# andrekuros/Multi-UAV-TA-gym-env

Hardware: AMD Instinct MI355X
Metric: env-steps/sec at N parallel envs, WPS_hard 16x32; 1/2/4/8 GPU (higher is better)
Workload: dtype f64

## Files before the change

### multi-uav-ta-gym-env_amd/csrc/muavta_state.h

```cpp
#pragma once
#include <stdint.h>

#include "../../include/muavta.h"


enum {
  MUAVTA_ERR_NONE = 0,
  MUAVTA_ERR_TASK_SLOTS = 1,
  MUAVTA_ERR_QUEUE = 2,
  MUAVTA_ERR_EVENTS = 3,
  MUAVTA_ERR_PENDING = 4,
  MUAVTA_ERR_POSITION = 5,
  MUAVTA_ERR_ESCORTS = 6,
  MUAVTA_ERR_LSAP = 7,
};

enum { TF_ESCORT = 1, TF_COUNTED = 2, TF_REACHED = 4, TF_ELIGIBLE = 8, TF_DEADLINE = 16,
       TF_KNOWN_ALL = 32  };

struct DevParams {
  int32_t n_agents, n_tasks , max_tasks , n_threats;
  int32_t n_agent_groups, agent_type[MUAVTA_MAX_GROUPS], agent_count[MUAVTA_MAX_GROUPS];
  int32_t n_task_groups, task_type[MUAVTA_MAX_GROUPS], task_count[MUAVTA_MAX_GROUPS];
  int32_t n_threat_groups, threat_type[MUAVTA_MAX_GROUPS], threat_count[MUAVTA_MAX_GROUPS];
  int32_t max_time_steps, multiple_tasks_per_agent, early_terminate, capability_mask, saturate_mask,
      include_time_windows, threat_delay, hard_windows, window_length, burst_mode, burst_size,
      dual_region_bursts, share_knowledge, escort_enabled, num_obstacles, random_init_pos,
      escort_required_agents , commit_horizon;
  uint32_t escort_mask;
  double speed[7];
  double threat_prob;
  double reward_norm_factor;
  double sense_sq_bound;
  double fail_rate, arrival_rate, dynamic_idle_penalty, sense_radius, miss_penalty, on_time_bonus,
      reassign_penalty, escort_radius, escort_requirement, escort_intercept_radius, mutual_support_radius;
  double rw[8];
  double escort_sq_bound;
  double inv_mts, inv_max_tasks;
  int32_t slot_cap;
  int32_t rw_plain;
};

template <int A_, int T_, int H_, int R_, int E_, int Q_, bool REGC_ = false, bool OTFC_ = false, bool SLIM_ = false, bool TIMES_LDS_ = false>
struct Tile {
  static constexpr bool TIMES_LDS = TIMES_LDS_;
  static constexpr bool SLIM = SLIM_;
  static constexpr bool REGC = REGC_;
  static constexpr bool OTFC = OTFC_;
  static constexpr bool NO_COST_TILE = REGC_ || OTFC_;
  static constexpr int A = A_;
  static constexpr int T = T_;
  static constexpr int H = H_;
  static constexpr int R = R_;
  static constexpr int E = E_;
  static constexpr int Q = Q_;
  static constexpr int KW = (T_ + 31) / 32;
  static constexpr int MIN_WAVES = A_ > 32 ? 2 : 4;
  static_assert(A_ <= 64 && T_ <= 128 && H_ <= 64, "ids of agents / slots / threats are stored in int8");
};

template <int A> struct KnowMask { typedef uint64_t type; };
template <> struct KnowMask<16> { typedef uint16_t type; };
template <> struct KnowMask<24> { typedef uint32_t type; };
template <int A> struct BucketMask { typedef unsigned long long type; };
template <> struct BucketMask<16> { typedef uint32_t type; };
template <> struct BucketMask<24> { typedef uint32_t type; };

typedef int8_t i8;
typedef int16_t i16;
typedef uint8_t u8;

template <int A, int T, bool HERE> struct QueueSide {
  double a_nfx[A], a_nfy[A], a_nft[A];
  double t_org[T], t_done[T];
  double area[3][3];
};
template <int A, int T> struct QueueSide<A, T, false> {};

template <int T, bool HERE> struct TaskTimes {
  double t_init[T], t_dtime[T];
};
template <int T> struct TaskTimes<T, false> {};

template <int T> struct TaskReqs {
  double t_cur[6][T], t_alloc[6][T];
};
template <class TL>
struct alignas(16) EnvCold : QueueSide<TL::A, TL::T, TL::SLIM>, TaskReqs<TL::T>, TaskTimes<TL::T, !TL::TIMES_LDS> {
  enum { A = TL::A, T = TL::T, Q = TL::Q };
  double a_qtime[A][Q];
  double obst[8][3];
};

template <class TL>
struct alignas(16) EnvState : QueueSide<TL::A, TL::T, !TL::SLIM>, TaskTimes<TL::T, TL::TIMES_LDS> {
  enum { A = TL::A, T = TL::T, H = TL::H, R = TL::R, E = TL::E, Q = TL::Q, KW = TL::KW };
  double a_px[A], a_py[A];
  double a_dist[A];
  double a_caps[6][A];
  double t_px[T], t_py[T];
  double h_px[H], h_py[H];
  typename BucketMask<A>::type t_bucket[T];
  uint32_t known[A][KW];
  uint32_t free_slots[KW];
  i16 act_index[A];
  i16 a_qid[A][Q];
  i16 a_task_start[A], a_fail[A], a_last_id[A], a_commit[A];
  i16 a_gone[A];
  i16 t_id[T];
  i16 t_created[T], t_deadline[T], t_prot_id[T];
  i16 h_task_id[H], h_tdeadline[H];
  i16 ev_arg[E], dev_arg[E];
  i16 pend_time[R], pend_id[R];
  i16 esc_id[A], esc_pid[A];
  typename KnowMask<A>::type pend_know[R];
  i8 a_qslot[A][Q];
  i8 a_qlen[A];
  i8 a_state[A], a_acap[A], a_type[A], a_name[A], a_reeval[A], a_last_slot[A];
  i8 t_status[T], t_type[T], t_required[T];
  u8 t_flags[T], t_elig[T];
  i8 t_threat[T];
  i8 t_prot_agent[T], t_prot_slot[T];
  i8 t_ndet[T];
  u8 t_order[T];
  u8 open_slot[T];
  u8 t_row[T];
  i8 h_status[H];
  i8 h_target[H], h_mission[H], h_intercept[H];
  i8 h_task_slot[H], h_det_slot[H], h_acap[H], h_type[H], h_group[H];
  u8 h_tflags[H];
  u8 h_order[H];
  i8 g_next[MUAVTA_MAX_GROUPS], g_end[MUAVTA_MAX_GROUPS];
  u8 ev_tag[E];
  u8 dev_tag[E];
  u8 pend_slot[R];
  i8 esc_agent[A], esc_slot[A], esc_pslot[A];
  i8 act_agent[A], act_slot[A];
  unsigned long long esc_mask;
  double F_Reward, total_distance, last_reward, step_reward;
  double r_time_penalty, r_alloc;
  int32_t time_steps, conclusion_time, n_order, n_open, n_active_threats, n_events, n_dev, n_pending, n_escorts, n_act;
  int32_t next_task_id, n_reached, n_retired_empty_buckets;
  int32_t n_reallocations, n_task_switches, n_arrivals, n_missed_windows, n_on_time, n_windowed_tasks,
      idle_reserve_steps, burst_region_toggle, escort_requests, escort_completed, escort_failed,
      escort_required_steps, escort_covered_steps, protection_breaches, threats_intercepted, recon_losses,
      escort_losses, mutual_support_engagements, protected_rec_completed;
  int32_t pending_reset, terminated, truncated, error, did_reset;
  int32_t last_plan_step, n_replans, n_calls;
  int32_t gate_step;
  uint32_t rng_idx[4];
  uint32_t rng_win[4][8];
  uint32_t rng_win_at[4];
  int32_t times_dirty;
  int32_t obs_rows;
  int32_t list_stale;
};

#ifndef MUAVTA_TIMES_LDS
#define MUAVTA_TIMES_LDS 1
#endif
typedef Tile<16, 40, 16, 48, 40, 10, true, false, false, MUAVTA_TIMES_LDS != 0> Tile16;
#ifndef MUAVTA_TILE24_SLIM
#define MUAVTA_TILE24_SLIM 1
#endif
typedef Tile<24, 48, 24, 88, 32, 12, true, false, MUAVTA_TILE24_SLIM != 0> Tile24;
typedef Tile<64, 128, 48, 128, 96, 12, true, true> Tile64;

#define MUAVTA_REL_ROW 29
#define MUAVTA_RNG_STREAMS 4
#define MUAVTA_RNG_WORDS 1248
```

### multi-uav-ta-gym-env_amd/csrc/sim/step.inc

```
  DEV double np_sum_wave(const double* d, int n) {
    double res;
    if (n < 8) {
      res = 0.;
      for (int i = 0; i < n; i++) res += d[i];
      return res;
    }
    const int body = n - (n % 8);
    double r = 0.;
    if (lane < 8) {
      r = d[lane];
      for (int i = 8 + lane; i < body; i += 8) r += d[i];
    }
    r = r + dpp_xchg(r, 0);
    r = r + dpp_xchg(r, 1);
    r = r + dpp_xchg(r, 2);
    res = readlane_f64(r, 0);
    for (int i = body; i < n; i++) res += d[i];
    return res;
  }

  DEV double np_sum_lanes16(double d, int n_) {
    const int n = __builtin_amdgcn_readfirstlane(n_);
    double res;
    if (n < 8) {
      res = 0.;
      for (int i = 0; i < n; i++) res += readlane_f64(d, i);
      return res;
    }
    const int body = n - (n % 8);
    double r = d;
    if (body == 16) {
      const int lo = __builtin_amdgcn_update_dpp(0, __double2loint(d), 0x108, 0xf, 0xf, true);
      const int hi = __builtin_amdgcn_update_dpp(0, __double2hiint(d), 0x108, 0xf, 0xf, true);
      r = d + __hiloint2double(hi, lo);
    }
    r = r + dpp_xchg(r, 0);
    r = r + dpp_xchg(r, 1);
    r = r + dpp_xchg(r, 2);
    res = readlane_f64(r, 0);
    for (int i = body; i < n; i++) res += readlane_f64(d, i);
    return res;
  }

  DEV void step(bool write_obs_flag) {
    PROF(0);
    in_step = true;
    uint32_t rng_words = 0;
    if (!ABL(0)) { rng_refill(); rng_words = rng_prefetch_issue(); }
    PROF(1);
    double prev_x = 0, prev_y = 0;
    if (lane < P.n_agents) { prev_x = S.a_px[lane]; prev_y = S.a_py[lane]; }
    lds_sync();
    double r_action = 0, r_distance = 0, r_quality = 0, r_squality = 0;
    {
      const int nev = S.n_events;
      for (int k = lane; k < nev; k += WG) { S.dev_tag[k] = S.ev_tag[k]; S.dev_arg[k] = S.ev_arg[k]; }
      tnow += 1;
      if (lane == 0) { S.step_reward = 0; S.time_steps = tnow; S.n_dev = nev; S.n_events = 0; }
      lds_sync();
      int last_arg = -1000;
      bool last_changed = true;
      if (!ABL(1))
      for (int k = 0; k < nev; k++)
        if (S.dev_tag[k] == MUAVTA_EV_RESET_ALLOCATION) {
          const int arg = S.dev_arg[k];
          if (arg == last_arg && !last_changed) continue;
          last_changed = release_all_tasks_coop(arg);
          last_arg = arg;
        }
    }
    PROF(2);
    if (!ABL(2))
    for (;;) {
      if (S.n_act > 0 && !apply_actions_parallel(r_action, r_distance, r_squality)) {
        precompute_actions();
        lds_sync();
        PROF(33);
        if (lane == 0) step_serial_a(r_action, r_distance, r_quality, r_squality);
        cold_sync();
      }
      if (!more_agent || stage_more() == 0) break;
    }
    PROF(3);
    for (int start = ABL(3) ? P.n_agents : 0; start < P.n_agents;) {
      bool popped = false;
      const int first = move_parallel(start, popped);
      if (popped) cold_sync(); else lds_sync();
      PROF(26);
#ifdef MUAVTA_PROF
      PROF_COUNT(40, 1000); if (first < P.n_agents) PROF_COUNT(41, 1000);
#endif
      if (first >= P.n_agents) break;
      if (lane == 0) step_serial_move(first, first + 1, r_quality);
      cold_sync();
      PROF(4);
      start = first + 1;
    }
    double dist_sum = 0.0;
    if (!ABL(4)) {
      double d = 0.0;
      if (lane < P.n_agents) {
        double dx = S.a_px[lane] - prev_x, dy = S.a_py[lane] - prev_y;
        d = fsqrt(dx * dx + dy * dy);
        S.a_dist[lane] += d;
        if constexpr (A > 16) X.u[lane] = d;
      }
      if constexpr (A <= 16) dist_sum = np_sum_lanes16(d, P.n_agents);
      else { lds_sync(); dist_sum = np_sum_wave(X.u, P.n_agents); }
    }
    if (!ABL(0)) rng_prefetch_commit(rng_words);
    PROF(5);
    if (!ABL(5)) {
    precompute_threat_targets();
    if (lane == 0) step_serial_b(dist_sum);
    lds_sync();
    }
    if (!ABL(5))
    {
      unsigned long long livemask = 0ull;
      if (lane == 0) X.retarget_h = -1;
      if (!P.escort_enabled) {
        const unsigned long long em = update_threats_parallel(0, livemask, true);
        lds_sync();
        PROF(23);
        PROF_COUNT(54, 1000);
        if (em) {
          PROF_COUNT(55, 1000 * __popcll(em));
          for (unsigned long long m = em; m; m &= m - 1ull) {
            if (lane == 0) update_threats_serial(__ffsll((long long)m) - 1, livemask);
            lds_sync();
            resolve_retarget();
          }
        }
      } else
      for (int start = 0;;) {
        const int first = (int)update_threats_parallel(start, livemask, false);
        lds_sync();
        PROF(23);
        PROF_COUNT(54, 1000);
        if (first >= S.n_active_threats) break;
        PROF_COUNT(55, 1000);
        if (lane == 0) update_threats_serial(first, livemask);
        lds_sync();
        resolve_retarget();
        start = first + 1;
      }
      if (lane == 0) step_serial_b2();
    }
    lds_sync();
    if (!ABL(6)) {
    if (P.escort_enabled) sync_escorts_coop();
    PROF(6);
    sense_parallel();
    lds_sync();
    }
    PROF(7);
    if (!ABL(7))
    {
      bool due = false, expiring = false, idle = false, resp = false, blocking = false;
      if (!ABL(12)) for (int k = lane; k < S.n_pending; k += WG) due |= tnow >= S.pend_time[k];
      auto scan_slots = [&]() {
        expiring = false; blocking = false;
        for (int k = lane; k < S.n_order; k += WG) {
          const int s = S.t_order[k];
          const int fl = S.t_flags[s], st = S.t_status[s], dl = S.t_deadline[s], ty = S.t_type[s];
          expiring |= (fl & TF_DEADLINE) && st != 2 && tnow > dl;
          blocking |= !((fl & TF_ESCORT) || ty == MUAVTA_DET || ty == MUAVTA_HOLD || st == 2);
        }
        idle = false; resp = false;
        if (lane < P.n_agents && S.a_state[lane] != -1) { idle = S.a_qlen[lane] == 0; resp = !idle; }
      };
      if (!ABL(12)) scan_slots();
      const bool any_due = __ballot(due) != 0ull;
      const bool any_exp = P.hard_windows && __ballot(expiring) != 0ull;
      PROF(28);
      if (any_due || any_exp) process_lists_coop(any_due, any_exp);
      lds_sync();
      PROF(29);
      if (any_exp) scan_slots();
      const int n_idle = __popcll(__ballot(idle));
      const bool responding = __ballot(resp) != 0ull;
      const bool all_done_tasks = __ballot(blocking) == 0ull;
      PROF(32);
      if (!ABL(11) && lane == 0) step_serial_c(r_action, r_distance, r_quality, r_squality, n_idle, responding, all_done_tasks);
    }
    lds_sync();
    PROF(8);
    if (!ABL(8)) finish_step_parallel(true);
    PROF(9);
  }

  DEV void displacement(double px, double py, double ux, double uy, double speed, double& ddx, double& ddy) {
    double avx, avy;
    avoid_obstacles(px, py, ux, uy, avx, avy);
    double mx = ux + avx, my = uy + avy;
    norm_vector(mx, my);
    ddx = mx * speed; ddy = my * speed;
  }
  DEV int move_parallel(int start, bool& popped) {
    const int a = lane;
    const bool in_fleet = a >= start && a < P.n_agents;
    const int ai = in_fleet ? a : 0;
    const int st0 = S.a_state[ai], fail_at = S.a_fail[ai], ts0 = S.a_task_start[ai], qlen = S.a_qlen[ai], reeval = S.a_reeval[ai];
    const int atype = S.a_type[ai];
    const int last_id = S.a_last_id[ai], last_slot = S.a_last_slot[ai], head_id_ = S.a_qid[ai][0], head_slot = S.a_qslot[ai][0];
    double px = S.a_px[ai], py = S.a_py[ai];
    const bool live = in_fleet && st0 != -1;
    int cid = 0, cs = -1;
    if (reeval) { cid = last_id; cs = last_slot; }
    else if (qlen > 0) { cid = head_id_; cs = head_slot; }
    const int csi = cs >= 0 ? cs : 0;
    const int tid_at = S.t_id[csi], tstat = S.t_status[csi], ty = S.t_type[csi];
    const double tpx = S.t_px[csi], tpy = S.t_py[csi];
    bool evt = false, pop_head = false;
    int new_st = 0, new_ts = 0;
    double ddx = 0.0, ddy = 0.0;
    if (live) {
      if (fail_at == tnow) {
        evt = true;
      } else {
        const double speed = speed_of(atype);
        new_st = st0; new_ts = ts0;
        const bool retired = cid != 0 && (!(cs >= 0 && tid_at == cid) || tstat == 2);
        const bool to_task = cid != 0 && !retired;
        const bool idle_check = new_st == 0 && !reeval && qlen == 0;
        const bool to_base = !to_task && (idle_check || new_st == 3);
        if (retired) pop_head = true;
        if (to_task || to_base) {
          const double tx = to_task ? tpx : BASE_X, ty_ = to_task ? tpy : BASE_Y;
          const double dx = tx - px, dy = ty_ - py;
          const double dist = norm2(dx, dy);
          double ux = 0, uy = 0;
          const bool zero = to_task ? (fabs(dist) < 1e-12) : (dist == 0);
          if (!zero) { const double r = frcp_nr(dist); ux = fdiv_r(dx, dist, r); uy = fdiv_r(dy, dist, r); }
          double ndx, ndy;
          displacement(px, py, ux, uy, speed, ndx, ndy);
          if (to_task) {
            const double engage = engage_range(atype);
            if (new_st == 1) {
              if (ty == MUAVTA_INT) {
                if (dist < engage) evt = true;
                else { ddx = ndx; ddy = ndy; }
              } else if (dist < speed) {
                new_st = 2; new_ts = tnow;
                px = tpx; py = tpy;
              } else { ddx = ndx; ddy = ndy; }
            } else if (new_st == 2) {
              if (ty == MUAVTA_INT && dist >= engage) new_st = 1;
              if (new_ts == -1) {
                new_ts = tnow;
                px = tpx; py = tpy;
              } else if ((tnow - new_ts) >= task_duration(ty) && ty != MUAVTA_HOLD && ty != MUAVTA_DEF &&
                         ty != MUAVTA_INT && ty != MUAVTA_DET) {
                evt = true;
              }
            }
          } else {
            if (idle_check && dist > speed + 5) new_st = 3;
            if (new_st == 3) {
              if (dist < speed + 5) new_st = 0;
              else { ddx = ndx; ddy = ndy; }
            }
          }
        }
      }
    }
    const unsigned long long em = __ballot(evt);
    const int first = em ? __ffsll((long long)em) - 1 : P.n_agents;
    PROF(34);
    popped = __ballot(live && a < first && pop_head) != 0ull;
    if (live && a < first) {
      if (pop_head) {
        des_allocate(a, cid);
        S.a_reeval[a] = 0;
        S.a_last_id[a] = -1; S.a_last_slot[a] = -1;
      }
      S.a_state[a] = new_st;
      S.a_task_start[a] = new_ts;
      px = px + ddx; py = py + ddy;
      S.a_px[a] = fmin(fmax(px, 0.0), AREA_W);
      S.a_py[a] = fmin(fmax(py, 0.0), AREA_H);
    }
    return first;
  }

  DEV double* act_f(int k) { return X.cost + k * A; }
  DEV void precompute_actions() {
    cold_sync();
    const int k = lane;
    if (k >= S.n_act) return;
    const int a = S.act_agent[k], s = S.act_slot[k];
    X.remaining[k] = -1;
    if (a < 0 || s < 0 || S.a_state[a] == -1) return;
    const double px = S.a_px[a], py = S.a_py[a], tx = S.t_px[s], ty = S.t_py[s];
    double d_old = 0;
    if (S.a_qlen[a] > 0) { const int hs = S.a_qslot[a][0]; d_old = norm2(px - S.t_px[hs], py - S.t_py[hs]); }
    act_f(0)[k] = d_old;
    act_f(1)[k] = norm2(px - tx, py - ty);
    act_f(2)[k] = fdiv(norm2(qs().a_nfx[a] - tx, qs().a_nfy[a] - ty), speed_of(S.a_type[a]));
    const int n = S.a_qlen[a];
    double total;
    if (n >= 1) { const int ps = S.a_qslot[a][n - 1]; total = norm2(tx - S.t_px[ps], ty - S.t_py[ps]); }
    else total = norm2(tx - px, ty - py);
    act_f(3)[k] = -div_coord(total);
    bool dup = false;
#pragma clang loop unroll(disable) vectorize(disable)
    for (int q = 0; q < k; q++) dup |= S.act_agent[q] == a;
    if (!dup) X.remaining[k] = a;
  }
```

### multi-uav-ta-gym-env_amd/csrc/sim/world.inc

```
  DEV bool threat_spawn_step() const { return tnow > 40 && tnow % 10 == 0; }
  DEV void precompute_threat_targets() {
    if (!threat_spawn_step() || P.dual_region_bursts) return;
    const int nA = P.n_agents;
    for (int g = 0; g < P.n_threat_groups; g++) {
      const int start = S.g_next[g], left = S.g_end[g] - start;
      int cnt = P.burst_mode ? (P.burst_size < left ? P.burst_size : left) : (left > 0 ? 1 : 0);
      if (cnt <= 0) continue;
      const int chunk = Scratch<TL>::COSTN / nA;
      for (int c0 = 0; c0 < cnt; c0 += chunk) {
        const int cn = cnt - c0 < chunk ? cnt - c0 : chunk;
        for (int p = lane; p < cn * nA; p += WG) {
          const int c = p / nA, a = p - c * nA, h = start + c0 + c;
          const int st = S.a_state[a];
          X.cost[p] = (h < H && st != -1 && st != 4) ? norm2(S.a_px[a] - S.h_px[h], S.a_py[a] - S.h_py[h]) : __builtin_huge_val();
        }
        lds_sync();
        for (int c = lane; c < cn; c += WG) {
          double minF = __builtin_huge_val(), minW = __builtin_huge_val();
          int cF = -1, cW = -1;
          for (int a = 0; a < nA; a++) {
            const double d = X.cost[c * nA + a];
            const int st = S.a_state[a];
            if (st != -1 && st != 4) {
              if (is_fighter(S.a_type[a])) { if (d < minF) { minF = d; cF = a; } }
              else { if (d < minW) { minW = d; cW = a; } }
            }
          }
          if (start + c0 + c < H) X.roundT[start + c0 + c] = cW >= 0 ? cW : cF;
        }
        lds_sync();
      }
    }
  }
  DEV void generate_threat() {
    if (!threat_spawn_step()) return;
    for (int g = 0; g < P.n_threat_groups; g++) {
      int left = S.g_end[g] - S.g_next[g];
      if (left > 0 && threat_spawn_step()) {
        if (rnd(ST_AGENT) < P.threat_prob) {
          int n_spawn = 1;
          if (P.burst_mode) n_spawn = P.burst_size < left ? P.burst_size : left;
          for (int bi = 0; bi < n_spawn; bi++) {
            if (S.g_next[g] >= S.g_end[g]) break;
            int h = S.g_next[g]++;
            if (h >= H) { fail(MUAVTA_ERR_TASK_SLOTS); break; }
            if (P.dual_region_bursts) {
              double mid = AREA_W * 0.5;
              double wide = fmax(AREA_W / 10, 40.0);
              double x;
              if ((S.burst_region_toggle + bi) % 2 == 0) x = uniform(ST_AGENT, wide, mid - wide);
              else x = uniform(ST_AGENT, mid + wide, AREA_W - wide);
              S.h_px[h] = x;
            }
            const int tgt = P.dual_region_bursts ? closest_agent(S.h_px[h], S.h_py[h]) : X.roundT[h];
            S.h_target[h] = tgt;
            S.h_mission[h] = tgt;
            int ty = S.h_type[h];
            double attack = threat_attack(ty), defence = threat_defence(ty);
            int s = new_task(S.h_px[h], S.h_py[h], MUAVTA_INT, 2.0);
            if (s >= 0) {
              C.t_cur[MUAVTA_ATT][s] = defence * 2;
              C.t_cur[MUAVTA_DEF][s] = attack * 2;
              obs_static_clear();
              S.t_threat[s] = h;
              S.t_created[s] = tnow;
              if (ty == MUAVTA_T1) { S.t_required[s] = 2; S.t_flags[s] |= TF_ELIGIBLE; S.t_elig[s] = P.escort_mask; }
              S.h_task_id[h] = S.t_id[s];
              S.h_task_slot[h] = s;
            }
            S.h_status[h] = 1;
            S.h_order[S.n_active_threats++] = h;
            C.t_cur[5][S.h_det_slot[h]] -= 1.0;
            if (s >= 0) {
              register_dynamic(s);
              push_event(MUAVTA_EV_NEW_THREAT, S.t_id[s]);
            }
            push_event(MUAVTA_EV_RESET_ALLOCATION, MUAVTA_INT);
            S.pending_reset = 1;
          }
          if (P.dual_region_bursts && n_spawn > 0) S.burst_region_toggle = (S.burst_region_toggle + 1) % 2;
        }
      }
    }
  }

  DEV void threat_task_retire(int h, bool success) {
    int s = S.h_task_slot[h];
    if (ref_valid(S.h_task_id[h], s)) { S.t_status[s] = 2; mark_outcome_slot(s, success); }
    else mark_outcome(S.h_tflags[h], S.h_tdeadline[h], success);
  }

  DEV void handle_threat_engagement(int h) {
    int primary = S.h_target[h];
    int mission = S.h_mission[h] >= 0 ? S.h_mission[h] : primary;
    int n_def = 0;
    int16_t* defs = X.remaining;
    double* defd = X.v;
    if (P.escort_enabled && mission >= 0 && is_recon(S.a_type[mission])) {
      n_def = escort_fighters_near(mission, P.mutual_support_radius, defs, defd);
      if (n_def > 0) {
        primary = defs[0];
        S.h_target[h] = primary;
        S.h_intercept[h] = primary;
      }
    }
    if (primary < 0) return;
    const int hty = S.h_type[h];
    const double t_att = threat_attack(hty), t_def = threat_defence(hty), t_rng = engage_range(hty);
    double attDiff, defDiff, engageDiff;
    if (n_def >= 2) {
      S.mutual_support_engagements++;
      double att_sum = 0, def_sum = 0, eng_sum = 0;
      for (int k = 0; k < n_def; k++) att_sum += S.a_caps[2][defs[k]];
      for (int k = 0; k < n_def; k++) def_sum += S.a_caps[3][defs[k]];
      for (int k = 0; k < n_def; k++) eng_sum += engage_range(S.a_type[defs[k]]);
      eng_sum = eng_sum / (double)n_def;
      attDiff = att_sum / fmax(t_att, 1e-6);
      defDiff = def_sum / fmax(t_def, 1e-6);
      engageDiff = eng_sum / fmax(t_rng, 1e-6);
    } else {
      attDiff = S.a_caps[2][primary] / fmax(t_att, 1e-6);
      defDiff = S.a_caps[3][primary] / fmax(t_def, 1e-6);
      engageDiff = engage_range(S.a_type[primary]) / fmax(t_rng, 1e-6);
    }
    double avg_diff = (attDiff + defDiff + engageDiff) / 3;
    double prob = avg_diff / (avg_diff + 1);
    double r = rnd(ST_AGENT);
    if (r < prob) {
      S.h_status[h] = 2;
      threat_task_retire(h, true);
      S.threats_intercepted++;
      S.a_acap[primary] -= 1;
      if (S.a_acap[primary] <= 0) S.a_caps[3][primary] = 0;
      if (S.a_qlen[primary] > 0 && S.a_qid[primary][0] == S.h_task_id[h]) task_done(primary, S.h_task_id[h], MUAVTA_INT);
      S.step_reward += 1.0;
    } else {
      S.h_acap[h] -= 1;
      S.a_acap[primary] -= 1;
      if (S.a_acap[primary] <= 0) {
        S.a_caps[3][primary] = 0;
        bool was_recon = is_recon(S.a_type[primary]);
        bool was_escort = escort_type(S.a_type[primary]);
        out_of_service(primary);
        if (was_recon) { S.recon_losses++; S.protection_breaches++; retire_escort_for(primary, true); }
        else if (was_escort) S.escort_losses++;
        S.step_reward -= 1.0;
      }
      if (S.h_acap[h] <= 0) {
        S.h_status[h] = 0;
        threat_task_retire(h, false);
      } else {
        X.retarget_h = h;
      }
    }
  }

  DEV unsigned long long update_threats_parallel(int start, unsigned long long& livemask, bool all_at_once) {
    static_assert(H <= 64, "one threat per lane");
    const int n = S.n_active_threats;
    const int k = lane;
    const int h = k < n ? (int)S.h_order[k] : 0;
    const int hst = S.h_status[h], hty = S.h_type[h], slot = S.h_task_slot[h], task_id = S.h_task_id[h], htf = S.h_tflags[h];
    int tgt = S.h_target[h], icpt = S.h_intercept[h];
    const int hmis = S.h_mission[h];
    const double px = S.h_px[h], py = S.h_py[h];
    bool active = k < n && hst != 2;
    if (start == 0) livemask = __ballot(active);
    active = k >= start && k < n && ((livemask >> k) & 1ull);
    const int sli = slot >= 0 ? slot : 0;
    const int t_id_at = S.t_id[sli], t_stat = S.t_status[sli], t_fl = S.t_flags[sli];
    bool evt = false;
    double npx = 0, npy = 0;
    bool live_task = false;
    if (P.escort_enabled) {
      const int mission = hmis >= 0 ? hmis : tgt;
      const int mi = mission >= 0 ? mission : 0;
      const bool need = active && !(hst == 0 || tgt < 0) && mission >= 0 && S.a_state[mi] != -1 && is_recon(S.a_type[mi]);
      int e0, cnt;
      closest_escort_lanes(need, mi, P.escort_intercept_radius, e0, cnt);
      if (need) {
        if (cnt == 0) { tgt = mission; icpt = -1; }
        else { tgt = e0; icpt = e0; }
      }
    }
    if (active) {
      const double speed = speed_of(hty);
      if (hst == 0 || tgt < 0) {
        npx = px + speed * 0.0;
        npy = py + speed * -1.0;
      } else {
        const double ax = S.a_px[tgt], ay = S.a_py[tgt];
        double dx = ax - px, dy = ay - py;
        norm_vector(dx, dy);
        npx = px + speed * dx;
        npy = py + speed * dy;
        if (norm2(ax - npx, ay - npy) < engage_range(hty)) evt = true;
      }
      live_task = slot >= 0 && t_id_at == task_id;
      if (npy <= 0) {
        if (live_task) evt |= (t_stat != 2) || ((t_fl & TF_DEADLINE) && !(t_fl & TF_COUNTED));
        else evt |= (htf & TF_DEADLINE) && !(htf & TF_COUNTED);
      }
    }
    const unsigned long long em = __ballot(evt);
    const int first = em ? __ffsll((long long)em) - 1 : n;
    if (active && (all_at_once ? !evt : k < first)) {
      S.h_px[h] = npx; S.h_py[h] = npy;
      S.h_target[h] = tgt; S.h_intercept[h] = icpt;
      if (live_task) { S.t_px[slot] = npx; S.t_py[slot] = npy; }
    }
    return all_at_once ? em : (unsigned long long)first;
  }
  DEV void update_threats_serial(int first, unsigned long long livemask) {
    const int n = first + 1 < S.n_active_threats ? first + 1 : S.n_active_threats;
    for (int k = first; k < n; k++) {
      if (!((livemask >> k) & 1ull)) continue;
      int h = S.h_order[k];
      const double speed = speed_of(S.h_type[h]);
      if (S.h_status[h] == 0 || S.h_target[h] < 0) {
        S.h_px[h] = S.h_px[h] + speed * 0.0;
        S.h_py[h] = S.h_py[h] + speed * -1.0;
      } else {
        if (P.escort_enabled) {
          int mission = S.h_mission[h] >= 0 ? S.h_mission[h] : S.h_target[h];
          if (mission >= 0 && S.a_state[mission] != -1 && is_recon(S.a_type[mission])) {
            int cnt;
            int e0 = closest_escort(mission, P.escort_intercept_radius, &cnt);
            if (cnt == 0) { S.h_target[h] = mission; S.h_intercept[h] = -1; }
            else { S.h_target[h] = e0; S.h_intercept[h] = e0; }
          }
        }
        int tg = S.h_target[h];
        double dx = S.a_px[tg] - S.h_px[h], dy = S.a_py[tg] - S.h_py[h];
        norm_vector(dx, dy);
        S.h_px[h] = S.h_px[h] + speed * dx;
        S.h_py[h] = S.h_py[h] + speed * dy;
        if (norm2(S.a_px[tg] - S.h_px[h], S.a_py[tg] - S.h_py[h]) < engage_range(S.h_type[h])) handle_threat_engagement(h);
      }
      int s = S.h_task_slot[h];
      bool live = ref_valid(S.h_task_id[h], s);
      if (live) { S.t_px[s] = S.h_px[h]; S.t_py[s] = S.h_py[h]; }
      if (S.h_py[h] <= 0) threat_task_retire(h, false);
    }
  }

  DEV void inject_dynamic_arrivals() {
    if (P.arrival_rate <= 0 || tnow < 5) return;
    if (rnd(ST_TGT) >= P.arrival_rate) return;
    if (S.next_task_id - 1 >= P.max_tasks - 1) return;
    int ty = randbelow(ST_TGT, 2) == 0 ? MUAVTA_ATT : MUAVTA_REC;
    int sel = (int)randbelow(ST_MISSION, 3);
    double x, y;
    if (P.dual_region_bursts) {
      double mid = AREA_W * 0.5, wide = 40.0;
      if (rnd(ST_TGT) < 0.5) x = uniform(ST_TGT, wide, mid - wide);
      else x = uniform(ST_TGT, mid + wide, AREA_W - wide);
      y = uniform(ST_TGT, AREA_H * 0.2, AREA_H * 0.8);
    } else {
      random_position(ST_TGT, 20, 3, true, sel, true, x, y);
    }
    int s = new_task(x, y, ty, 1.0);
    S.n_arrivals++;
    if (s >= 0) {
      S.t_created[s] = tnow;
      register_dynamic(s);
      push_event(MUAVTA_EV_NEW_THREAT, S.t_id[s]);
    }
    push_event(MUAVTA_EV_RESET_ALLOCATION, ty);
    S.pending_reset = 1;
  }

  DEV void sync_escorts() {
    for (int a = 0; a < P.n_agents; a++) {
      if (S.a_state[a] == -1 || !is_recon(S.a_type[a])) continue;
      if (S.a_qlen[a] == 0) continue;
      int cid = S.a_qid[a][0], cs = S.a_qslot[a][0];
      if (ref_retired(cid, cs)) continue;
      if (S.t_type[cs] == MUAVTA_REC && !has_escort(a)) create_escort_for(a, cs);
    }
    int n = S.n_escorts;
    int16_t* snap = X.row4col;
    for (int k = 0; k < n; k++) snap[k] = S.esc_agent[k];
    for (int k = 0; k < n; k++) {
      int recon = snap[k];
      int kk = escort_lookup(recon);
      if (kk < 0) continue;
      int es = S.esc_slot[kk];
      int rid = S.esc_pid[kk], rs = S.esc_pslot[kk];
      bool dead = S.a_state[recon] == -1;
      bool idle = S.a_qlen[recon] == 0 || S.a_state[recon] == 0 || S.a_state[recon] == 3;
      bool rec_done = ref_retired(rid, rs);
      bool wrong_task = S.a_qlen[recon] > 0 && S.a_qid[recon][0] != rid;
      if (dead || idle || rec_done || wrong_task) { retire_escort_entry(kk, dead); continue; }
      if (ref_valid(S.esc_id[kk], es)) { S.t_px[es] = S.a_px[recon]; S.t_py[es] = S.a_py[recon]; }
      S.escort_required_steps++;
      int cnt;
      closest_escort(recon, P.escort_radius, &cnt);
      if (cnt > 0) S.escort_covered_steps++;
    }
  }

  DEV void sync_escorts_coop() {
    {
      const int a = lane;
      bool need = false;
      int cs = -1;
      if (a < P.n_agents && S.a_state[a] != -1 && is_recon(S.a_type[a]) && S.a_qlen[a] > 0) {
        const int cid = S.a_qid[a][0];
        cs = S.a_qslot[a][0];
        need = !ref_retired(cid, cs) && S.t_type[cs] == MUAVTA_REC && !has_escort(a);
      }
      unsigned long long nm = __ballot(need);
      if (nm) {
        if (lane == 0) {
          while (nm) {
            const int b = __ffsll((long long)nm) - 1;
            nm &= nm - 1ull;
            create_escort_for(b, S.a_qslot[b][0]);
          }
        }
        lds_sync();
      }
    }
    PROF(59);
    const int n = S.n_escorts;
    if (n == 0) return;
    int recon = -1, es = -1, eid = -1, rid = -1, rs = -1;
    bool retire = false, dead = false, esc_live = false, esc_here = false;
    auto decide = [&]() {
      if (lane < n) {
        dead = S.a_state[recon] == -1;
        const bool idle = S.a_qlen[recon] == 0 || S.a_state[recon] == 0 || S.a_state[recon] == 3;
        const bool rec_done = ref_retired(rid, rs);
        const bool wrong_task = S.a_qlen[recon] > 0 && S.a_qid[recon][0] != rid;
        retire = dead || idle || rec_done || wrong_task;
      }
    };
    if (lane < n) {
      recon = S.esc_agent[lane]; es = S.esc_slot[lane]; eid = S.esc_id[lane];
      rid = S.esc_pid[lane]; rs = S.esc_pslot[lane];
      esc_here = ref_valid(eid, es);
      esc_live = esc_here && S.t_status[es] != 2;
    }
    decide();
    const bool recon_escorts = (P.escort_mask & ((1u << MUAVTA_R1) | (1u << MUAVTA_R2))) != 0u;
    const unsigned long long all = n >= 64 ? ~0ull : ((1ull << n) - 1ull);
    unsigned long long rm = __ballot(retire), todo = all;
    PROF_COUNT(56, 1000); PROF_COUNT(57, 1000 * n);
    while (todo) {
      PROF_COUNT(58, 1000);
      const unsigned long long low = todo & (0ull - todo);
      const unsigned long long nextr = rm & todo;
      const unsigned long long seg = nextr ? (todo & ((nextr & (0ull - nextr)) - 1ull)) : todo;
      if (seg) {
        const bool fighter = lane < P.n_agents && S.a_state[lane] != -1 && escort_type(S.a_type[lane]) && S.a_qlen[lane] > 0;
        const int head = fighter ? S.a_qid[lane][0] : -1;
        const unsigned long long live_m = __ballot(esc_live);
        int myk = -1, my_recon = 0;
        for (unsigned long long m = seg & live_m; m; m &= m - 1ull) {
          const int k = __ffsll((long long)m) - 1;
          const int ek = __builtin_amdgcn_readlane(eid, k), rk = __builtin_amdgcn_readlane(recon, k);
          if (head == ek) { myk = k; my_recon = rk; }
        }
        bool near = false;
        if (fighter && myk >= 0) {
          const double dx = S.a_px[lane] - S.a_px[my_recon], dy = S.a_py[lane] - S.a_py[my_recon];
          near = fma(dy, dy, dx * dx) <= P.escort_sq_bound;
        }
        unsigned long long cov = 0ull;
        const int neark = near ? myk : -2;
        if (__ballot(near) != 0ull)
          for (unsigned long long m = seg & live_m; m; m &= m - 1ull) {
            const int k = __ffsll((long long)m) - 1;
            if (__builtin_amdgcn_ballot_w64(neark == k) != 0ull) cov |= 1ull << k;
          }
        if ((seg >> lane) & 1ull) {
          if (esc_here) { S.t_px[es] = S.a_px[recon]; S.t_py[es] = S.a_py[recon]; }
        }
        if (lane == 0) { S.escort_required_steps += __popcll(seg); S.escort_covered_steps += __popcll(cov); }
        todo &= ~seg;
        lds_sync();
        PROF(60);
      } else {
        const int k = __ffsll((long long)low) - 1;
        const int rk = __builtin_amdgcn_readlane(recon, k), ek = __builtin_amdgcn_readlane(eid, k);
        const bool dk = (__ballot(dead) >> k) & 1ull;
        retire_escort_coop(rk, dk);
        (void)ek;
        todo &= ~low;
        if (recon_escorts && todo) {
          lds_sync();
          decide();
          rm = __ballot(retire);
        }
        PROF(61);
      }
    }
  }

  DEV void sense_parallel() {
    if (P.sense_radius <= 0) return;
    const int nA = P.n_agents, nO = S.n_order;
    int16_t* cand = X.roundT;
    int nc = 0;
    for (int base = 0; base < nO; base += WG) {
      const int k = base + lane;
      int s = -1;
      bool c = false;
      if (k < nO) {
        s = S.t_order[k];
        const int fl = S.t_flags[s];
        c = S.t_status[s] != 2 && !(fl & TF_KNOWN_ALL) && (S.t_created[s] > 0 || (fl & TF_DEADLINE));
      }
      const unsigned long long m = __ballot(c);
      if (c) cand[nc + prefix_count(m)] = s;
      nc += __popcll(m);
    }
    if (nc == 0) return;
    lds_sync();
    int aw = 1;
    while (aw < nA) aw <<= 1;
    const int a = lane & (aw - 1), sub = lane / aw, stride = WG / aw;
    if (!(a < nA && S.a_state[a] != -1)) return;
    const double ax = S.a_px[a], ay = S.a_py[a];
    for (int k = sub; k < nc; k += stride) {
      const int s = cand[k];
      if ((S.known[a][s >> 5] >> (s & 31)) & 1u) continue;
      const double dx = ax - S.t_px[s], dy = ay - S.t_py[s];
      if (fma(dy, dy, dx * dx) <= P.sense_sq_bound) atomicOr(&S.known[a][s >> 5], 1u << (s & 31));
    }
  }


  DEV void process_lists_coop(bool any_due, bool any_exp) {
    const unsigned long long below = (1ull << lane) - 1ull;
    if (any_due) {
      const int n = S.n_pending;
      int w = 0;
      for (int base = 0; base < n; base += WG) {
        const int k = base + lane;
        int pt = 0, pid = -1, psl = 0;
        typename KnowMask<A>::type pk = 0;
        if (k < n) { pt = S.pend_time[k]; pid = S.pend_id[k]; psl = S.pend_slot[k]; pk = S.pend_know[k]; }
        const bool due = k < n && tnow >= pt;
        const unsigned long long dm = __ballot(due), km = __ballot(k < n && !due);
        if (P.share_knowledge) {
          for (unsigned long long m = dm; m; m &= m - 1ull) {
            const int b = __ffsll((long long)m) - 1;
            const int id = __builtin_amdgcn_readlane(pid, b), sl = __builtin_amdgcn_readlane(psl, b);
            if (ref_valid(id, sl)) {
              if (lane < P.n_agents) S.known[lane][sl >> 5] |= 1u << (sl & 31);
              if (lane == 0) S.t_flags[sl] |= TF_KNOWN_ALL;
            } else if (lane < P.n_agents) {
              const unsigned long long kn = (unsigned long long)S.pend_know[base + b];
              S.a_gone[lane] += !((kn >> lane) & 1ull);
            }
          }
        }
        lds_sync();
        if (k < n && !due) {
          const int d = w + prefix_count(km);
          S.pend_time[d] = pt; S.pend_id[d] = pid; S.pend_slot[d] = (uint8_t)psl; S.pend_know[d] = pk;
        }
        w += __popcll(km);
      }
      if (lane == 0) S.n_pending = w;
      lds_sync();
    }
    if (any_exp) {
      const int n = S.n_order;
      for (int base = 0; base < n; base += WG) {
        const int k = base + lane;
        int sl = -1;
        bool ex = false;
        if (k < n) {
          sl = S.t_order[k];
          ex = (S.t_flags[sl] & TF_DEADLINE) && S.t_status[sl] != 2 && tnow > S.t_deadline[sl];
        }
        for (unsigned long long m = __ballot(ex); m; m &= m - 1ull) {
          const int b = __ffsll((long long)m) - 1;
          const int s_ = __builtin_amdgcn_readlane(sl, b);
          const int id = S.t_id[s_];
          const unsigned long long hm = __ballot(lane < P.n_agents && S.a_qlen[lane] > 0 && S.a_qid[lane][0] == id);
          if (lane == 0) {
            S.t_status[s_] = 2;
            mark_outcome_slot(s_, false);
            if (!(S.t_flags[s_] & TF_REACHED)) { S.t_flags[s_] |= TF_REACHED; S.n_reached++; }
            for (unsigned long long h = hm; h; h &= h - 1ull) desallocate_all(__ffsll((long long)h) - 1);
          }
          lds_sync();
        }
      }
    }
  }
  DEV void step_serial_c(double action_reward, double distance_reward, double quality_reward, double S_quality_reward,
                         int idle, bool responding, bool all_done_tasks) {
    const int irs = S.idle_reserve_steps, pr = S.pending_reset, ntid = S.next_task_id, ct = S.conclusion_time;
    const double time_penaulty = S.r_time_penalty, alloc_reward = S.r_alloc, step_reward = S.step_reward, FR = S.F_Reward;
    PROF(36);
    const unsigned long long any_bits = (unsigned long long)__double_as_longlong(action_reward) | (unsigned long long)__double_as_longlong(distance_reward) |
                                        (unsigned long long)__double_as_longlong(quality_reward) | (unsigned long long)__double_as_longlong(S_quality_reward) |
                                        (unsigned long long)__double_as_longlong(alloc_reward) | (unsigned long long)__double_as_longlong(time_penaulty) |
                                        (unsigned long long)__double_as_longlong(step_reward);
    const bool quiet_reward = P.rw_plain && any_bits == 0ull;
    double total = 0.0;
    if (!quiet_reward)
    total = P.rw[0] * action_reward + P.rw[1] * distance_reward + P.rw[2] * quality_reward + P.rw[3] * S_quality_reward +
                   P.rw[4] * (double)P.n_tasks * 0.0 + P.rw[5] * alloc_reward + P.rw[6] * time_penaulty + P.rw[7] * step_reward;
    PROF(37);
    const double shared = quiet_reward ? 0.0
                          : P.reward_norm_factor != 0 ? fdiv(fdiv(total, P.reward_norm_factor), (double)P.max_time_steps)
                                                      : total / P.reward_norm_factor / (double)P.max_time_steps;
    PROF(38);
    const bool all_done = (ntid > 1) && all_done_tasks;
    const bool timed_out = (tnow >= P.max_time_steps) && (P.max_time_steps > 0);
    const bool done = timed_out || (P.early_terminate && all_done);
    S.idle_reserve_steps = irs + idle;
    if (pr && responding) S.pending_reset = 0;
    if (all_done && ct > P.max_time_steps) S.conclusion_time = tnow;
    S.terminated = P.early_terminate && all_done && !timed_out;
    S.truncated = timed_out;
    S.last_reward = done ? FR : shared;
  }

  DEV void finish_step_parallel(bool gc) {
    if (gc) {
      const int n = S.n_order, no = S.n_open;
      bool ret = false, diff = false;
      for (int k = lane; k < n; k += WG) {
        const int s = S.t_order[k];
        ret |= S.t_status[s] == 2;
        diff |= k >= no || (int)S.open_slot[k] != s;
      }
      const bool any_ret = __ballot(ret) != 0ull;
      if (!any_ret && no == n && __ballot(diff) == 0ull) {
        if (lane == 0) { S.n_act = 0; S.list_stale = 0; }
        lds_sync();
        return;
      }
#ifdef MUAVTA_PROF
      PROF_COUNT(30, 1000); if (any_ret) PROF_COUNT(31, 1000);
#endif
      if (any_ret) {
        if (rel_log) cold_sync();
        uint32_t* refmask = reinterpret_cast<uint32_t*>(X.path);
        uint32_t* relmask = refmask + KW;
        if (lane < 2 * KW) refmask[lane] = 0;
        lds_sync();
        if (lane < P.n_agents && S.a_state[lane] != -1) {
          const int ql = S.a_qlen[lane];
          for (int k = 0; k < ql; k++) {
            const int qs = S.a_qslot[lane][k];
            if (ref_valid(S.a_qid[lane][k], qs)) atomicOr(&refmask[qs >> 5], 1u << (qs & 31));
          }
        }
        lds_sync();
        for (int k = lane; k < n; k += WG) {
          const int s = S.t_order[k];
          if (S.t_status[s] == 2 && !((refmask[s >> 5] >> (s & 31)) & 1u)) {
            release_slot_record(s);
            atomicOr(&relmask[s >> 5], 1u << (s & 31));
          }
        }
        lds_sync();
        if (lane < P.n_agents) {
          int gone = 0;
          for (int w = 0; w < KW; w++) {
            const uint32_t m = relmask[w];
            if (m) { const uint32_t old = S.known[lane][w]; gone += __popc(old & m); S.known[lane][w] = old & ~m; }
          }
          if (gone) S.a_gone[lane] += gone;
        }
        if (lane < KW) S.free_slots[lane] |= relmask[lane];
        lds_sync();
      }
      PROF(35);
    }
    {
      const int n = S.n_order, no_old = S.n_open;
      int w = 0, no = 0;
      bool moved = false;
      for (int base = 0; base < n; base += WG) {
        const int k = base + lane;
        int s = -1;
        bool alive = false, open = false;
        if (k < n) {
          s = S.t_order[k];
          alive = S.t_id[s] >= 0;
          open = alive && S.t_status[s] != 2;
        }
        const unsigned long long am = __ballot(alive), om = __ballot(open);
        const unsigned long long below = (1ull << lane) - 1ull;
        lds_sync();
        if (alive) S.t_order[w + prefix_count(am)] = s;
        if (open) {
          const int row = no + prefix_count(om);
          moved |= row >= no_old || (int)S.open_slot[row] != s;
          S.open_slot[row] = s; S.t_row[s] = (uint8_t)row;
        }
        w += __popcll(am);
        no += __popcll(om);
      }
      const bool list_changed = __ballot(moved) != 0ull || no != no_old;
      if (lane == 0) { S.n_order = w; S.n_open = no; S.n_act = 0; S.list_stale = 0; if (list_changed) obs_static_clear(); }
    }
    lds_sync();
  }
```

Baseline: 272.1 million.

## Fuse per-step slot list scans into a single wave pass in step tail

Adds a SlotScan pass that walks the task order list once per step and computes, with wave ballots, the sense candidates, due/expiring/blocking flags, retirement/diff flags and idle-agent counts. The step tail, sensing and finish_step_parallel then reuse these results instead of each rescanning the slot list in LDS. It is enabled by default for Tile16 only through a template flag. The scan is redone after expiry processing. The risk is stale scan state if intermediate stages (escort sync, sensing) change slot status or order before finish_step reads the cached any_ret/any_diff.

```diff
diff --git a/multi-uav-ta-gym-env_amd/csrc/muavta_state.h b/multi-uav-ta-gym-env_amd/csrc/muavta_state.h
--- a/multi-uav-ta-gym-env_amd/csrc/muavta_state.h
+++ b/multi-uav-ta-gym-env_amd/csrc/muavta_state.h
@@ -41,8 +41,9 @@
   int32_t rw_plain;
 };
 
-template <int A_, int T_, int H_, int R_, int E_, int Q_, bool REGC_ = false, bool OTFC_ = false, bool SLIM_ = false, bool TIMES_LDS_ = false>
+template <int A_, int T_, int H_, int R_, int E_, int Q_, bool REGC_ = false, bool OTFC_ = false, bool SLIM_ = false, bool TIMES_LDS_ = false, bool SCAN_ONCE_ = false>
 struct Tile {
+  static constexpr bool SCAN_ONCE = SCAN_ONCE_;
   static constexpr bool TIMES_LDS = TIMES_LDS_;
   static constexpr bool SLIM = SLIM_;
   static constexpr bool REGC = REGC_;
@@ -159,12 +160,15 @@
 #ifndef MUAVTA_TIMES_LDS
 #define MUAVTA_TIMES_LDS 1
 #endif
-typedef Tile<16, 40, 16, 48, 40, 10, true, false, false, MUAVTA_TIMES_LDS != 0> Tile16;
+#ifndef MUAVTA_SCAN_ONCE
+#define MUAVTA_SCAN_ONCE 1
+#endif
+typedef Tile<16, 40, 16, 48, 40, 10, true, false, false, MUAVTA_TIMES_LDS != 0, (MUAVTA_SCAN_ONCE & 1) != 0> Tile16;
 #ifndef MUAVTA_TILE24_SLIM
 #define MUAVTA_TILE24_SLIM 1
 #endif
-typedef Tile<24, 48, 24, 88, 32, 12, true, false, MUAVTA_TILE24_SLIM != 0> Tile24;
-typedef Tile<64, 128, 48, 128, 96, 12, true, true> Tile64;
+typedef Tile<24, 48, 24, 88, 32, 12, true, false, MUAVTA_TILE24_SLIM != 0, false, (MUAVTA_SCAN_ONCE & 2) != 0> Tile24;
+typedef Tile<64, 128, 48, 128, 96, 12, true, true, false, false, (MUAVTA_SCAN_ONCE & 4) != 0> Tile64;
 
 #define MUAVTA_REL_ROW 29
 #define MUAVTA_RNG_STREAMS 4
diff --git a/multi-uav-ta-gym-env_amd/csrc/sim/step.inc b/multi-uav-ta-gym-env_amd/csrc/sim/step.inc
--- a/multi-uav-ta-gym-env_amd/csrc/sim/step.inc
+++ b/multi-uav-ta-gym-env_amd/csrc/sim/step.inc
@@ -148,6 +148,7 @@
       if (lane == 0) step_serial_b2();
     }
     lds_sync();
+    if constexpr (TL::SCAN_ONCE) { step_tail_one_pass(r_action, r_distance, r_quality, r_squality); return; }
     if (!ABL(6)) {
     if (P.escort_enabled) sync_escorts_coop();
     PROF(6);
@@ -187,6 +188,31 @@
     lds_sync();
     PROF(8);
     if (!ABL(8)) finish_step_parallel(true);
+    PROF(9);
+  }
+  DEV void step_tail_one_pass(double r_action, double r_distance, double r_quality, double r_squality) {
+    SlotScan sc;
+    if (!ABL(6) && P.escort_enabled) sync_escorts_coop();
+    PROF(6);
+    slot_pass(sc, true, !ABL(6));
+    if (!ABL(6)) sense_parallel(sc.nc);
+    lds_sync();
+    PROF(7);
+    if (!ABL(7))
+    {
+      const bool any_due = !ABL(12) && sc.any_due;
+      const bool any_exp = !ABL(12) && P.hard_windows && sc.any_expiring;
+      PROF(28);
+      if (any_due || any_exp) process_lists_coop(any_due, any_exp);
+      lds_sync();
+      PROF(29);
+      if (any_exp) slot_pass(sc, false, false);
+      PROF(32);
+      if (!ABL(11) && lane == 0) step_serial_c(r_action, r_distance, r_quality, r_squality, sc.n_idle, sc.responding, !sc.any_blocking);
+    }
+    lds_sync();
+    PROF(8);
+    if (!ABL(8)) finish_step_parallel(true, &sc);
     PROF(9);
   }
 
diff --git a/multi-uav-ta-gym-env_amd/csrc/sim/world.inc b/multi-uav-ta-gym-env_amd/csrc/sim/world.inc
--- a/multi-uav-ta-gym-env_amd/csrc/sim/world.inc
+++ b/multi-uav-ta-gym-env_amd/csrc/sim/world.inc
@@ -398,11 +398,64 @@
     }
   }
 
-  DEV void sense_parallel() {
+  struct SlotScan {
+    int nc = 0;
+    int n_idle = 0;
+    bool any_due = false;
+    bool any_expiring = false;
+    bool any_blocking = false;
+    bool responding = false;
+    bool any_ret = false;
+    bool any_diff = false;
+  };
+  DEV void slot_pass(SlotScan& sc, bool first, bool sense) {
+    const int nO = S.n_order, no = S.n_open, np = S.n_pending;
+    const int ai = lane < A ? lane : A - 1;
+    const int ast = S.a_state[ai], aql = S.a_qlen[ai];
+    bool due = false;
+    if (first) {
+      if constexpr (R <= WG) { due = lane < np && tnow >= S.pend_time[lane < R ? lane : R - 1]; }
+      else for (int k = lane; k < np; k += WG) due |= tnow >= S.pend_time[k];
+    }
+    const bool want_cand = first && sense && P.sense_radius > 0;
+    int16_t* cand = X.roundT;
+    int nc = 0;
+    bool expiring = false, blocking = false, ret = false, diff = false;
+#pragma unroll
+    for (int base = 0; base < T; base += WG) {
+      if (base > 0 && base >= nO) break;
+      const int k = base + lane, ki = k < T ? k : T - 1;
+      const bool in = k < nO;
+      const int s_ = S.t_order[ki], os = S.open_slot[ki];
+      const int s = s_ < T ? s_ : T - 1;
+      const int fl = S.t_flags[s], st = S.t_status[s], dl = S.t_deadline[s], ty = S.t_type[s], cr = S.t_created[s];
+      expiring |= in && (fl & TF_DEADLINE) && st != 2 && tnow > dl;
+      blocking |= in && !((fl & TF_ESCORT) || ty == MUAVTA_DET || ty == MUAVTA_HOLD || st == 2);
+      ret |= in && st == 2;
+      diff |= in && (k >= no || os != s);
+      if (want_cand) {
+        const bool c = in && st != 2 && !(fl & TF_KNOWN_ALL) && (cr > 0 || (fl & TF_DEADLINE));
+        const unsigned long long m = __ballot(c);
+        if (c) cand[nc + prefix_count(m)] = s;
+        nc += __popcll(m);
+      }
+    }
+    const bool live = lane < P.n_agents && ast != -1;
+    if (first) { sc.nc = nc; sc.any_due = __ballot(due) != 0ull; }
+    sc.any_expiring = __ballot(expiring) != 0ull;
+    sc.any_blocking = __ballot(blocking) != 0ull;
+    sc.any_ret = __ballot(ret) != 0ull;
+    sc.any_diff = no != nO || __ballot(diff) != 0ull;
+    sc.n_idle = __popcll(__ballot(live && aql == 0));
+    sc.responding = __ballot(live && aql != 0) != 0ull;
+  }
+
+  DEV void sense_parallel(int nc_scan = 0) {
     if (P.sense_radius <= 0) return;
     const int nA = P.n_agents, nO = S.n_order;
     int16_t* cand = X.roundT;
     int nc = 0;
+    if constexpr (TL::SCAN_ONCE) nc = nc_scan; else
     for (int base = 0; base < nO; base += WG) {
       const int k = base + lane;
       int s = -1;
@@ -523,7 +576,14 @@
     S.last_reward = done ? FR : shared;
   }
 
-  DEV void finish_step_parallel(bool gc) {
+  DEV void finish_step_parallel(bool gc, const SlotScan* sc = nullptr) {
+    if constexpr (TL::SCAN_ONCE) {
+      if (gc && sc && !sc->any_ret && !sc->any_diff) {
+        if (lane == 0) { S.n_act = 0; S.list_stale = 0; }
+        lds_sync();
+        return;
+      }
+    }
     if (gc) {
       const int n = S.n_order, no = S.n_open;
       bool ret = false, diff = false;
```

After: 279.6 million, median of 6. 1.03x the previous value.
